# mohsij/spacecraft-pose-estimation

Measured on AMD Instinct MI355X. Metric: poses/sec end-to-end (HRNet+PnP) at batch 256; keypoint/pose err vs ref, higher is better.
Workload: dtype bf16

## Files before the change

### spacecraft-pose-estimation_amd/csrc/bottleneck.hip

```cpp
#include "common.h"
#include "conv_device.h"
#include "conv_pipe_kernel.h"

namespace scpose {

namespace {

constexpr int kT = 16;
constexpr int kHW = kT + 2, kHPix = kHW * kHW;
constexpr int kCols1 = (kHPix + 15) / 16;
constexpr int kXS = (kHPix | 1) * 16;
constexpr int kT2S = (kT * kT | 1) * 16;
constexpr int kW1Bytes = 8 * 4 * 4 * 16 * 16;
constexpr int kW2LSteps = 13;
constexpr int kLds = 8 * kXS + 8 * kT2S + kW1Bytes + (64 + 64 + 256) * 4 + 16 + kW2LSteps * 4 * 1024;
constexpr int kW1BytesProj = 2 * 4 * 4 * 16 * 16;
constexpr int kLdsProj = 8 * kXS + 8 * kT2S + 2 * 8 * kT2S + kW1BytesProj + (64 + 64 + 256) * 4 + 16;

struct BneckLaunch {
  const void* in;
  const void* w1;
  const void* w2;
  const void* w3;
  const float* b1;
  const float* b2;
  const float* b3;
  void* out;
  uint32_t in_bytes, out_bytes;
  int32_t N, H, W;
  int32_t tiles_x, tiles_y, tiles_total, grid;
  uint32_t* sched;
  int32_t xcd_local;
  unsigned long long* dbg_buf;
};

inline int bneck_row_channel(int row) {
  const int q = row >> 2, reg = row & 3;
  return (q & 1) * 8 + (q >> 1) * 4 + reg;
}

}

template <int S, int E, typename F>
__device__ __forceinline__ void static_for_b(F&& f) {
  if constexpr (S < E) { f(std::integral_constant<int, S>{}); static_for_b<S + 1, E>(f); }
}

#ifndef SCPOSE_BNECK_EARLY
#define SCPOSE_BNECK_EARLY 2
#endif
#ifndef SCPOSE_BNECK_EARLY_PROJ
#define SCPOSE_BNECK_EARLY_PROJ 1
#endif
template <int DT, bool PROJ>
__global__ __launch_bounds__(512, 2) void bottleneck_kernel(const BneckLaunch p) {
  constexpr int EARLY = PROJ ? SCPOSE_BNECK_EARLY_PROJ : SCPOSE_BNECK_EARLY;
  constexpr int CINP = PROJ ? 8 : 32;
  constexpr int KA = CINP / 4;
  constexpr int KC = PROJ ? 4 : 2;
  constexpr int W1B = PROJ ? kW1BytesProj : kW1Bytes;
  extern __shared__ __attribute__((aligned(16))) char smem[];
  typedef typename DtOf<DT>::type T;
  typedef typename FragOf<T>::type frag_t;
  char* t1l = smem;
  char* t2l = t1l + 8 * kXS;
  char* xcl = t2l + 8 * kT2S;
  char* w1l = xcl + (PROJ ? 2 * 8 * kT2S : 0);

  const int tid = threadIdx.x, lane = tid & 63, wave = __builtin_amdgcn_readfirstlane(tid >> 6);
  const int q = lane >> 4, r = lane & 15, half = lane >> 5, psel = q & 1;
  const int ch = wave & 1, wq = wave >> 1;
  const int HW = p.H * p.W;
  const int tiles_per_img = p.tiles_x * p.tiles_y;

  for (int o = tid * 16; o < W1B; o += 512 * 16)
    *reinterpret_cast<u32x4*>(w1l + o) = *reinterpret_cast<const u32x4*>(static_cast<const char*>(p.w1) + o);
  frag_t w3f[KC][2];
#pragma unroll
  for (int s = 0; s < KC; ++s)
#pragma unroll
    for (int mb = 0; mb < 2; ++mb)
      w3f[s][mb] = *reinterpret_cast<const frag_t*>(static_cast<const char*>(p.w3) + ((((size_t)s * 16 + 2 * wave + mb) * 4 + q) * 16 + r) * 16);
  float* bl = reinterpret_cast<float*>(w1l + W1B);
  for (int e = tid; e < 64 + 64 + 256; e += 512) bl[e] = e < 64 ? p.b1[e] : e < 128 ? p.b2[e - 64] : p.b3[e - 128];
  const int qoff = q * kXS;
  const uint32_t w2vo = (uint32_t)(((2 * ch) * 4 + q) * 16 + r) * 16u;

  int* tq = reinterpret_cast<int*>(bl + 64 + 64 + 256);
  constexpr int W2L = PROJ ? 0 : kW2LSteps;
  char* w2ll = reinterpret_cast<char*>(tq) + 16;
  for (int o = tid * 16; o < W2L * 4 * 1024; o += 512 * 16)
    *reinterpret_cast<u32x4*>(w2ll + o) = *reinterpret_cast<const u32x4*>(static_cast<const char*>(p.w2) + o);
  const int xcd = xcc_id();
  auto claim = [&]() { return p.xcd_local ? tile_claim_xcd(p.sched, xcd, p.N, tiles_per_img) : tile_claim(p.sched + 9, p.tiles_total); };
  if (tid == 0) { tq[0] = claim(); tq[1] = tq[0] < 0 ? -1 : claim(); }
  __syncthreads();
  int t = tq[0], t_next = tq[1];
  auto decode = [&](int t, int& img, int& oy0, int& ox0) {
    img = t / tiles_per_img;
    const int rem = t - img * tiles_per_img;
    const int ty = rem / p.tiles_x;
    oy0 = ty * kT; ox0 = (rem - ty * p.tiles_x) * kT;
  };
  const buf_rsrc_t rs_in = make_buf(p.in, p.in_bytes), rs_out = make_buf(p.out, p.out_bytes), rs_w2 = make_buf(p.w2, 18u * 4 * 4 * 16 * 16);
  const uint32_t kstep_bytes = (uint32_t)(4 * HW) * 16u;

  const bool has_col2 = wave + 16 < kCols1;
  uint32_t vo[3];
  int cx[3] = {-1, -1, -1};
  auto locate = [&](int t) {
    int img, oy0, ox0;
    decode(t, img, oy0, ox0);
#pragma unroll
    for (int i = 0; i < 3; ++i) {
      const int slot = (wave + 8 * i) * 16 + r;
      const int my = slot / kHW, mx = slot - my * kHW;
      const int gy = oy0 - 1 + my, gx = ox0 - 1 + mx;
      const bool ok = slot < kHPix && gy >= 0 && gy < p.H && gx >= 0 && gx < p.W;
      vo[i] = ok ? (uint32_t)((img * CINP + q) * HW + gy * p.W + gx) * 16u : BUF_OOB;
      if constexpr (PROJ) cx[i] = (slot < kHPix && my >= 1 && my <= kT && mx >= 1 && mx <= kT) ? ((my - 1) * kT + mx - 1) * 16 : -1;
    }
  };
  u32x4 xr[KA][3];
  auto request = [&](auto sc) {
    constexpr int S = decltype(sc)::value;
    if constexpr (S < KA)
#pragma unroll
      for (int i = 0; i < 3; ++i)
        xr[S][i] = load16_buf(rs_in, vo[i], (uint32_t)S * kstep_bytes);
  };
  auto request_head = [&]() {
    request(std::integral_constant<int, 0>{}); request(std::integral_constant<int, 1>{});
    request(std::integral_constant<int, 2>{}); request(std::integral_constant<int, 3>{});
    request(std::integral_constant<int, 4>{}); request(std::integral_constant<int, 5>{});
    request(std::integral_constant<int, 6>{}); request(std::integral_constant<int, 7>{});
  };

  if (t >= 0) {
    locate(t);
    request_head();
  }
  asm volatile("s_waitcnt lgkmcnt(0)" ::: "memory");
  __builtin_amdgcn_s_barrier();

  unsigned long long tph[6] = {0, 0, 0, 0, 0, 0};
  auto now = [&]() -> unsigned long long { return SCP_DBG_BUF(p) ? __builtin_amdgcn_s_memtime() : 0ull; };
  int xbuf = 0;
  for (; t >= 0; t = t_next, t_next = tq[2], xbuf ^= 1) {
    int img, oy0, ox0;
    decode(t, img, oy0, ox0);
    const unsigned long long ts0 = now();
    int t_after = -1;
    if (tid == 0 && t_next >= 0) t_after = claim();

    frag_t w2f[18 - W2L][2];
    const uint32_t pl_bytes = (uint32_t)HW * 16u;
    auto out_off = [&](int cp) -> uint32_t {
      const int oy = oy0 + 2 * cp + half, ox = ox0 + r;
      return (oy < p.H && ox < p.W) ? (uint32_t)((img * 32 + psel) * HW + oy * p.W + ox) * 16u : BUF_OOB;
    };
    u32x4 rv[PROJ ? 1 : 8][2];
    {
      f32x4 acc[4][3];
#pragma unroll
      for (int mb = 0; mb < 4; ++mb) {
        const float4 bs = *reinterpret_cast<const float4*>(bl + mb * 16 + q * 4);
        acc[mb][0] = f32x4{bs.x, bs.y, bs.z, bs.w}; acc[mb][1] = acc[mb][0]; acc[mb][2] = acc[mb][0];
      }
      auto load_a = [&](int s, frag_t* a) {
#pragma unroll
        for (int mb = 0; mb < 4; ++mb) a[mb] = *reinterpret_cast<const frag_t*>(w1l + ((((s * 4 + mb) * 4 + q) * 16 + r) * 16));
      };
      frag_t fa[2][4];
      load_a(0, fa[0]);
      auto step = [&](auto sc) {
        constexpr int S = decltype(sc)::value;
        if constexpr (S + 1 < KA) load_a(S + 1, fa[(S + 1) & 1]);
        if constexpr (PROJ) {
#pragma unroll
          for (int i = 0; i < 3; ++i)
            if (cx[i] >= 0) *reinterpret_cast<u32x4*>(xcl + (xbuf * 8 + 4 * S + q) * kT2S + cx[i]) = xr[S][i];
        }
        __builtin_amdgcn_sched_barrier(0);
#pragma unroll
        for (int mb = 0; mb < 4; ++mb) {
          acc[mb][0] = mfma16<T>(fa[S & 1][mb], __builtin_bit_cast(frag_t, xr[S][0]), acc[mb][0]);
          acc[mb][1] = mfma16<T>(fa[S & 1][mb], __builtin_bit_cast(frag_t, xr[S][1]), acc[mb][1]);
          if (has_col2) acc[mb][2] = mfma16<T>(fa[S & 1][mb], __builtin_bit_cast(frag_t, xr[S][2]), acc[mb][2]);
        }
        __builtin_amdgcn_sched_barrier(0);
      };
      step(std::integral_constant<int, 0>{}); step(std::integral_constant<int, 1>{});
      if constexpr (KA > 2) {
        step(std::integral_constant<int, 2>{}); step(std::integral_constant<int, 3>{}); step(std::integral_constant<int, 4>{});
        step(std::integral_constant<int, 5>{}); step(std::integral_constant<int, 6>{}); step(std::integral_constant<int, 7>{});
      }
#pragma unroll
      for (int i = 0; i < 3; ++i) {
        const int slot = (wave + 8 * i) * 16 + r;
        const bool inimg = vo[i] != BUF_OOB;
#pragma unroll
        for (int mb = 0; mb < 4; ++mb) {
          uint2 o;
          o.x = relu2_16(pack2<T>(acc[mb][i][0], acc[mb][i][1]), 0u);
          o.y = relu2_16(pack2<T>(acc[mb][i][2], acc[mb][i][3]), 0u);
          if (!inimg) o = make_uint2(0u, 0u);
          if (slot < kHPix) *reinterpret_cast<uint2*>(t1l + (2 * mb + psel) * kXS + slot * 16 + 8 * (q >> 1)) = o;
        }
      }
      __builtin_amdgcn_sched_barrier(0);
#pragma unroll
      for (int s2 = W2L; s2 < 18; ++s2)
#pragma unroll
        for (int mb = 0; mb < 2; ++mb)
          w2f[s2 - W2L][mb] = __builtin_bit_cast(frag_t, load16_buf(rs_w2, w2vo, (uint32_t)((s2 * 4 + mb) * 1024)));
      __builtin_amdgcn_sched_barrier(0);
      if constexpr (!PROJ) {
#pragma unroll
        for (int cp = 0; cp < 8; ++cp) {
          const uint32_t o = out_off(cp);
#pragma unroll
          for (int mb = 0; mb < 2; ++mb) rv[cp][mb] = load16_buf(rs_in, o, (uint32_t)(2 * (2 * wave + mb)) * pl_bytes);
        }
        __builtin_amdgcn_sched_barrier(0);
      }
    }
    const unsigned long long ts1 = now();
    asm volatile("s_waitcnt lgkmcnt(0)" ::: "memory");
    __builtin_amdgcn_s_barrier();
    const unsigned long long ts2 = now();

    if constexpr (EARLY > 0) {
      __builtin_amdgcn_sched_barrier(0);
      if (t_next >= 0) locate(t_next);
      else { vo[0] = vo[1] = vo[2] = BUF_OOB; cx[0] = cx[1] = cx[2] = -1; }
      static_for_b<0, EARLY>([&](auto sc) { request(sc); });
      __builtin_amdgcn_sched_barrier(0);
    }
    constexpr int CC = PROJ ? 1 : 2;
#pragma unroll 1
    for (int c0 = 0; c0 < 4; c0 += CC) {
      f32x4 acc[2][CC];
#pragma unroll
      for (int mb = 0; mb < 2; ++mb) {
        const float4 bs = *reinterpret_cast<const float4*>(bl + 64 + (2 * ch + mb) * 16 + q * 4);
#pragma unroll
        for (int cc = 0; cc < CC; ++cc) acc[mb][cc] = f32x4{bs.x, bs.y, bs.z, bs.w};
      }
      const int px = r;
      const char* bq0 = t1l + ((wq + 4 * c0) * kHW + px) * 16 + qoff;
      const char* aq0 = w2ll + (2 * ch) * 1024 + lane * 16;
      auto k2imm = [](int s) { const int tap = s >> 1, ky = tap / 3, kx = tap - 3 * ky; return 4 * (s & 1) * kXS + (ky * kHW + kx) * 16; };
      frag_t bq[3][CC], aq[3][2];
      auto fetch = [&](auto sc) {
        constexpr int S = decltype(sc)::value;
        if constexpr (S < 18) {
#pragma unroll
          for (int cc = 0; cc < CC; ++cc) bq[S % 3][cc] = *reinterpret_cast<const frag_t*>(bq0 + cc * (4 * kHW * 16) + k2imm(S));
          if constexpr (S < W2L) {
            aq[S % 3][0] = *reinterpret_cast<const frag_t*>(aq0 + S * 4096);
            aq[S % 3][1] = *reinterpret_cast<const frag_t*>(aq0 + S * 4096 + 1024);
          }
        }
      };
      fetch(std::integral_constant<int, 0>{});
      fetch(std::integral_constant<int, 1>{});
      auto kstep = [&](auto sc) {
        constexpr int S = decltype(sc)::value;
        fetch(std::integral_constant<int, S + 2>{});
        __builtin_amdgcn_sched_barrier(0);
#pragma unroll
        for (int mb = 0; mb < 2; ++mb) {
          frag_t a;
          if constexpr (S < W2L) a = aq[S % 3][mb]; else a = w2f[S - W2L][mb];
#pragma unroll
          for (int cc = 0; cc < CC; ++cc) acc[mb][cc] = mfma16<T>(a, bq[S % 3][cc], acc[mb][cc]);
        }
        __builtin_amdgcn_sched_barrier(0);
      };
      kstep(std::integral_constant<int, 0>{}); kstep(std::integral_constant<int, 1>{}); kstep(std::integral_constant<int, 2>{});
      kstep(std::integral_constant<int, 3>{}); kstep(std::integral_constant<int, 4>{}); kstep(std::integral_constant<int, 5>{});
      kstep(std::integral_constant<int, 6>{}); kstep(std::integral_constant<int, 7>{}); kstep(std::integral_constant<int, 8>{});
      kstep(std::integral_constant<int, 9>{}); kstep(std::integral_constant<int, 10>{}); kstep(std::integral_constant<int, 11>{});
      kstep(std::integral_constant<int, 12>{}); kstep(std::integral_constant<int, 13>{}); kstep(std::integral_constant<int, 14>{});
      kstep(std::integral_constant<int, 15>{}); kstep(std::integral_constant<int, 16>{}); kstep(std::integral_constant<int, 17>{});
#pragma unroll
      for (int cc = 0; cc < CC; ++cc) {
        const int pix = (wq + 4 * (c0 + cc)) * kT + px;
#pragma unroll
        for (int mb = 0; mb < 2; ++mb) {
          uint2 o;
          o.x = relu2_16(pack2<T>(acc[mb][cc][0], acc[mb][cc][1]), 0u);
          o.y = relu2_16(pack2<T>(acc[mb][cc][2], acc[mb][cc][3]), 0u);
          *reinterpret_cast<uint2*>(t2l + (2 * (2 * ch + mb) + psel) * kT2S + pix * 16 + 8 * (q >> 1)) = o;
        }
      }
    }
    const unsigned long long ts3 = now();
    if (tid == 0) tq[2] = t_after;
    asm volatile("s_waitcnt lgkmcnt(0)" ::: "memory");
    __builtin_amdgcn_s_barrier();
    const unsigned long long ts4 = now();

    {
      __builtin_amdgcn_sched_barrier(0);
      if constexpr (EARLY == 0) {
        if (t_next >= 0) locate(t_next);
        else { vo[0] = vo[1] = vo[2] = BUF_OOB; cx[0] = cx[1] = cx[2] = -1; }
      }
      auto pair = [&](auto cpc) {
        constexpr int cp = decltype(cpc)::value;
        request(std::integral_constant<int, cp + EARLY>{});
        f32x4 acc[2][2];
#pragma unroll
        for (int mb = 0; mb < 2; ++mb) {
          const float4 bs = *reinterpret_cast<const float4*>(bl + 128 + (2 * wave + mb) * 16 + q * 4);
          acc[mb][0] = f32x4{bs.x, bs.y, bs.z, bs.w}; acc[mb][1] = acc[mb][0];
        }
        frag_t bc[KC][2];
#pragma unroll
        for (int s = 0; s < KC; ++s)
#pragma unroll
          for (int c = 0; c < 2; ++c)
            bc[s][c] = *reinterpret_cast<const frag_t*>((s < 2 ? t2l + (4 * s + q) * kT2S : xcl + (xbuf * 8 + 4 * (s - 2) + q) * kT2S) + ((2 * cp + c) * 16 + r) * 16);
        __builtin_amdgcn_sched_barrier(0);
#pragma unroll
        for (int s = 0; s < KC; ++s)
#pragma unroll
          for (int mb = 0; mb < 2; ++mb)
#pragma unroll
            for (int c = 0; c < 2; ++c) acc[mb][c] = mfma16<T>(w3f[s][mb], bc[s][c], acc[mb][c]);
        mfma_swap_pad(acc[0][0], acc[0][1], acc[1][0], acc[1][1]);
#pragma unroll
        for (int mb = 0; mb < 2; ++mb) {
          const f32x4 a0 = acc[mb][0], a1 = acc[mb][1];
          uint32_t a[4], b[4];
#pragma unroll
          for (int jj = 0; jj < 4; ++jj) { a[jj] = __float_as_uint(a0[jj]); b[jj] = __float_as_uint(a1[jj]); }
#pragma unroll
          for (int jj = 0; jj < 4; ++jj) {
            const auto sw = __builtin_amdgcn_permlane32_swap(a[jj], b[jj], false, false);
            a[jj] = sw[0]; b[jj] = sw[1];
          }
          float v[8];
#pragma unroll
          for (int jj = 0; jj < 4; ++jj) { v[jj] = __uint_as_float(a[jj]); v[4 + jj] = __uint_as_float(b[jj]); }
          if constexpr (!PROJ) {
          const u32x4 rr = rv[cp][mb];
          v[0] += from_bits<T>(rr[0] & 0xffff); v[1] += from_bits<T>(rr[0] >> 16);
          v[2] += from_bits<T>(rr[1] & 0xffff); v[3] += from_bits<T>(rr[1] >> 16);
          v[4] += from_bits<T>(rr[2] & 0xffff); v[5] += from_bits<T>(rr[2] >> 16);
          v[6] += from_bits<T>(rr[3] & 0xffff); v[7] += from_bits<T>(rr[3] >> 16);
          }
          u32x4 ov;
          ov[0] = relu2_16(pack2<T>(v[0], v[1]), 0u); ov[1] = relu2_16(pack2<T>(v[2], v[3]), 0u);
          ov[2] = relu2_16(pack2<T>(v[4], v[5]), 0u); ov[3] = relu2_16(pack2<T>(v[6], v[7]), 0u);
          store16_buf(rs_out, out_off(cp), (uint32_t)(2 * (2 * wave + mb)) * pl_bytes, ov);
        }
      };
      pair(std::integral_constant<int, 0>{}); pair(std::integral_constant<int, 1>{}); pair(std::integral_constant<int, 2>{});
      pair(std::integral_constant<int, 3>{}); pair(std::integral_constant<int, 4>{}); pair(std::integral_constant<int, 5>{});
      pair(std::integral_constant<int, 6>{}); pair(std::integral_constant<int, 7>{});
    }
    if (SCP_DBG_BUF(p)) {
      const unsigned long long ts5 = now();
      tph[0] += ts1 - ts0; tph[1] += ts2 - ts1; tph[2] += ts3 - ts2; tph[3] += ts4 - ts3; tph[4] += ts5 - ts4;
    }
  }
  if (tid == 0) { if (p.xcd_local) tile_retire_xcd(p.sched); else tile_retire(p.sched + 9); }
  if (SCP_DBG_BUF(p) && lane == 0)
    for (int k = 0; k < 6; ++k) SCP_DBG_BUF(p)[((size_t)blockIdx.x * 8 + wave) * 6 + k] = tph[k];
}

bool bottleneck_fusable(int cin, int cmid, int cout) { return (cin == 256 || cin == 64) && cmid == 64 && cout == 256; }

void bottleneck_pack(const float* w1, const float* w2, const float* w3, const float* wds, const float* b1, const float* b2, const float* b3,
                     const float* bds, int cin, int dtype,
                     std::vector<uint16_t>* pw1, std::vector<uint16_t>* pw2, std::vector<uint16_t>* pw3, std::vector<float>* pb) {
  const int ka = cin / 32, kc = wds ? 4 : 2;
  pw1->assign((size_t)ka * 4 * 4 * 16 * 8, 0);
  pw2->assign((size_t)18 * 4 * 4 * 16 * 8, 0);
  pw3->assign((size_t)kc * 16 * 4 * 16 * 8, 0);
  pb->assign(64 + 64 + 256, 0.f);
  for (int s = 0; s < ka; ++s)
    for (int m = 0; m < 4; ++m)
      for (int q = 0; q < 4; ++q)
        for (int r = 0; r < 16; ++r) {
          const int co = 16 * m + bneck_row_channel(r), plane = 4 * s + q;
          uint16_t* d = pw1->data() + ((((size_t)s * 4 + m) * 4 + q) * 16 + r) * 8;
          for (int j = 0; j < 8; ++j) d[j] = host_f32_to_16(w1[(size_t)co * cin + plane * 8 + j], dtype);
        }
  for (int s = 0; s < 18; ++s)
    for (int m = 0; m < 4; ++m)
      for (int q = 0; q < 4; ++q)
        for (int r = 0; r < 16; ++r) {
          const int co = 16 * m + bneck_row_channel(r);
          const int t = 4 * s + q, tap = t >> 3, plane = t & 7, ky = tap / 3, kx = tap % 3;
          uint16_t* d = pw2->data() + ((((size_t)s * 4 + m) * 4 + q) * 16 + r) * 8;
          for (int j = 0; j < 8; ++j) d[j] = host_f32_to_16(w2[((size_t)(co * 64 + plane * 8 + j) * 3 + ky) * 3 + kx], dtype);
        }
  for (int s = 0; s < kc; ++s)
    for (int m = 0; m < 16; ++m)
      for (int q = 0; q < 4; ++q)
        for (int r = 0; r < 16; ++r) {
          const int co = 16 * m + bneck_row_channel(r), plane = 4 * s + q;
          uint16_t* d = pw3->data() + ((((size_t)s * 16 + m) * 4 + q) * 16 + r) * 8;
          const float* src = plane < 8 ? w3 + (size_t)co * 64 + plane * 8 : wds + (size_t)co * 64 + (plane - 8) * 8;
          for (int j = 0; j < 8; ++j) d[j] = host_f32_to_16(src[j], dtype);
        }
  for (int pos = 0; pos < 64; ++pos) {
    const int co = (pos & ~15) + bneck_row_channel(pos & 15);
    (*pb)[pos] = b1[co]; (*pb)[64 + pos] = b2[co];
  }
  for (int pos = 0; pos < 256; ++pos) {
    const int co = (pos & ~15) + bneck_row_channel(pos & 15);
    (*pb)[128 + pos] = b3[co] + (bds ? bds[co] : 0.f);
  }
}

template <int DT, bool PROJ>
static int32_t bneck_launch_one(const BneckLaunch& L, hipStream_t stream) {
  auto kern = bottleneck_kernel<DT, PROJ>;
  constexpr int lds = PROJ ? kLdsProj : kLds;
  static LdsOptIn big;
  { const int32_t rc = lds_opt_in(reinterpret_cast<const void*>(kern), lds, &big); if (rc != SCPOSE_OK) return rc; }
  hipLaunchKernelGGL(kern, dim3(L.grid), dim3(512), lds, stream, L);
  SCP_CHECK_HIP(hipGetLastError());
  return SCPOSE_OK;
}

int32_t bottleneck_launch(const void* in, const void* w1, const void* w2, const void* w3, const float* bias, int N, int H, int W,
                          int cin, int dtype, void* out, uint32_t* sched, hipStream_t stream) {
  SCP_REQUIRE(sched, "bottleneck: null tile-queue words");
  const bool proj = cin == 64;
  SCP_REQUIRE(cin == 64 || cin == 256, "bottleneck: Cin = %d (64 or 256)", cin);
  const size_t in_frame = blocked_bytes(1, cin / 8, H, W), out_frame = blocked_bytes(1, 32, H, W);
  return for_frame_ranges(N, out_frame, [&](int n0, int n) -> int32_t {
    BneckLaunch L{};
    L.in = static_cast<const char*>(in) + (size_t)n0 * in_frame;
    L.out = static_cast<char*>(out) + (size_t)n0 * out_frame;
    L.w1 = w1; L.w2 = w2; L.w3 = w3; L.b1 = bias; L.b2 = bias + 64; L.b3 = bias + 128;
    L.in_bytes = (uint32_t)((size_t)n * in_frame); L.out_bytes = (uint32_t)((size_t)n * out_frame);
    L.N = n; L.H = H; L.W = W;
    L.tiles_x = (W + kT - 1) / kT; L.tiles_y = (H + kT - 1) / kT;
    L.tiles_total = n * L.tiles_x * L.tiles_y;
    L.grid = conv_device_cus() < L.tiles_total ? conv_device_cus() : L.tiles_total;
    L.sched = sched;
    { static const char* e = dev_env("SCPOSE_BNECK_GLOBALQ"); L.xcd_local = !(e && atoi(e)); }
    { static const char* e = dev_env("SCPOSE_BNECK_DBG"); L.dbg_buf = (kDevBuild && e && atoi(e)) ? conv_dbg_buffer(stream) : nullptr; if (L.dbg_buf) conv_dbg_set_grid(L.grid); }
    if (dtype == SCPOSE_DT_BF16) return proj ? bneck_launch_one<0, true>(L, stream) : bneck_launch_one<0, false>(L, stream);
    return proj ? bneck_launch_one<1, true>(L, stream) : bneck_launch_one<1, false>(L, stream);
  }, "bottleneck %d %dx%d", cin, H, W);
}

}
```

Before: 9994.

## Split bottleneck kernel into projection and identity paths, reuse centre input for residual

The fused bottleneck kernel is split into a projection variant and a specialised identity variant. The identity path splits input loads into centre pixels and halo ring, and keeps the centre registers for the residual add instead of reloading the input. It also prefetches the next tile's centre inputs inside the conv3 loop and stages w3 in LDS. Part of w2 moves from LDS to registers, and the conv2 wave/tile mapping changes to 4 output blocks by 2 row groups. The trade-off is more register pressure and a new LDS layout. An env override for grid size is also added.

```diff
diff --git a/spacecraft-pose-estimation_amd/csrc/bottleneck.hip b/spacecraft-pose-estimation_amd/csrc/bottleneck.hip
--- a/spacecraft-pose-estimation_amd/csrc/bottleneck.hip
+++ b/spacecraft-pose-estimation_amd/csrc/bottleneck.hip
@@ -12,8 +12,11 @@
 constexpr int kXS = (kHPix | 1) * 16;
 constexpr int kT2S = (kT * kT | 1) * 16;
 constexpr int kW1Bytes = 8 * 4 * 4 * 16 * 16;
-constexpr int kW2LSteps = 13;
-constexpr int kLds = 8 * kXS + 8 * kT2S + kW1Bytes + (64 + 64 + 256) * 4 + 16 + kW2LSteps * 4 * 1024;
+constexpr int kW3Bytes = 2 * 16 * 4 * 16 * 16;
+constexpr int kW2LSteps = 5;
+constexpr int kRing = 4 * kT + 4;
+constexpr int kLds = 8 * kXS + 8 * kT2S + kW1Bytes + (64 + 64 + 256) * 4 + 16 + kW2LSteps * 4 * 1024 + kW3Bytes;
+static_assert(kLds <= 160 * 1024, "identity Bottleneck: LDS");
 constexpr int kW1BytesProj = 2 * 4 * 4 * 16 * 16;
 constexpr int kLdsProj = 8 * kXS + 8 * kT2S + 2 * 8 * kT2S + kW1BytesProj + (64 + 64 + 256) * 4 + 16;
 
@@ -46,26 +49,23 @@
   if constexpr (S < E) { f(std::integral_constant<int, S>{}); static_for_b<S + 1, E>(f); }
 }
 
-#ifndef SCPOSE_BNECK_EARLY
-#define SCPOSE_BNECK_EARLY 2
-#endif
 #ifndef SCPOSE_BNECK_EARLY_PROJ
 #define SCPOSE_BNECK_EARLY_PROJ 1
 #endif
-template <int DT, bool PROJ>
-__global__ __launch_bounds__(512, 2) void bottleneck_kernel(const BneckLaunch p) {
-  constexpr int EARLY = PROJ ? SCPOSE_BNECK_EARLY_PROJ : SCPOSE_BNECK_EARLY;
-  constexpr int CINP = PROJ ? 8 : 32;
+template <int DT>
+__device__ __forceinline__ void bneck_first(const BneckLaunch& p) {
+  constexpr int EARLY = SCPOSE_BNECK_EARLY_PROJ;
+  constexpr int CINP = 8;
   constexpr int KA = CINP / 4;
-  constexpr int KC = PROJ ? 4 : 2;
-  constexpr int W1B = PROJ ? kW1BytesProj : kW1Bytes;
+  constexpr int KC = 4;
+  constexpr int W1B = kW1BytesProj;
   extern __shared__ __attribute__((aligned(16))) char smem[];
   typedef typename DtOf<DT>::type T;
   typedef typename FragOf<T>::type frag_t;
   char* t1l = smem;
   char* t2l = t1l + 8 * kXS;
   char* xcl = t2l + 8 * kT2S;
-  char* w1l = xcl + (PROJ ? 2 * 8 * kT2S : 0);
+  char* w1l = xcl + 2 * 8 * kT2S;
 
   const int tid = threadIdx.x, lane = tid & 63, wave = __builtin_amdgcn_readfirstlane(tid >> 6);
   const int q = lane >> 4, r = lane & 15, half = lane >> 5, psel = q & 1;
@@ -87,10 +87,6 @@
   const uint32_t w2vo = (uint32_t)(((2 * ch) * 4 + q) * 16 + r) * 16u;
 
   int* tq = reinterpret_cast<int*>(bl + 64 + 64 + 256);
-  constexpr int W2L = PROJ ? 0 : kW2LSteps;
-  char* w2ll = reinterpret_cast<char*>(tq) + 16;
-  for (int o = tid * 16; o < W2L * 4 * 1024; o += 512 * 16)
-    *reinterpret_cast<u32x4*>(w2ll + o) = *reinterpret_cast<const u32x4*>(static_cast<const char*>(p.w2) + o);
   const int xcd = xcc_id();
   auto claim = [&]() { return p.xcd_local ? tile_claim_xcd(p.sched, xcd, p.N, tiles_per_img) : tile_claim(p.sched + 9, p.tiles_total); };
   if (tid == 0) { tq[0] = claim(); tq[1] = tq[0] < 0 ? -1 : claim(); }
@@ -118,7 +114,7 @@
       const int gy = oy0 - 1 + my, gx = ox0 - 1 + mx;
       const bool ok = slot < kHPix && gy >= 0 && gy < p.H && gx >= 0 && gx < p.W;
       vo[i] = ok ? (uint32_t)((img * CINP + q) * HW + gy * p.W + gx) * 16u : BUF_OOB;
-      if constexpr (PROJ) cx[i] = (slot < kHPix && my >= 1 && my <= kT && mx >= 1 && mx <= kT) ? ((my - 1) * kT + mx - 1) * 16 : -1;
+      cx[i] = (slot < kHPix && my >= 1 && my <= kT && mx >= 1 && mx <= kT) ? ((my - 1) * kT + mx - 1) * 16 : -1;
     }
   };
   u32x4 xr[KA][3];
@@ -153,13 +149,12 @@
     int t_after = -1;
     if (tid == 0 && t_next >= 0) t_after = claim();
 
-    frag_t w2f[18 - W2L][2];
+    frag_t w2f[18][2];
     const uint32_t pl_bytes = (uint32_t)HW * 16u;
     auto out_off = [&](int cp) -> uint32_t {
       const int oy = oy0 + 2 * cp + half, ox = ox0 + r;
       return (oy < p.H && ox < p.W) ? (uint32_t)((img * 32 + psel) * HW + oy * p.W + ox) * 16u : BUF_OOB;
     };
-    u32x4 rv[PROJ ? 1 : 8][2];
     {
       f32x4 acc[4][3];
 #pragma unroll
@@ -176,11 +171,9 @@
       auto step = [&](auto sc) {
         constexpr int S = decltype(sc)::value;
         if constexpr (S + 1 < KA) load_a(S + 1, fa[(S + 1) & 1]);
-        if constexpr (PROJ) {
-#pragma unroll
-          for (int i = 0; i < 3; ++i)
-            if (cx[i] >= 0) *reinterpret_cast<u32x4*>(xcl + (xbuf * 8 + 4 * S + q) * kT2S + cx[i]) = xr[S][i];
-        }
+#pragma unroll
+        for (int i = 0; i < 3; ++i)
+          if (cx[i] >= 0) *reinterpret_cast<u32x4*>(xcl + (xbuf * 8 + 4 * S + q) * kT2S + cx[i]) = xr[S][i];
         __builtin_amdgcn_sched_barrier(0);
 #pragma unroll
         for (int mb = 0; mb < 4; ++mb) {
@@ -190,11 +183,8 @@
         }
         __builtin_amdgcn_sched_barrier(0);
       };
+      static_assert(KA == 2, "two k-steps of conv1");
       step(std::integral_constant<int, 0>{}); step(std::integral_constant<int, 1>{});
-      if constexpr (KA > 2) {
-        step(std::integral_constant<int, 2>{}); step(std::integral_constant<int, 3>{}); step(std::integral_constant<int, 4>{});
-        step(std::integral_constant<int, 5>{}); step(std::integral_constant<int, 6>{}); step(std::integral_constant<int, 7>{});
-      }
 #pragma unroll
       for (int i = 0; i < 3; ++i) {
         const int slot = (wave + 8 * i) * 16 + r;
@@ -210,20 +200,11 @@
       }
       __builtin_amdgcn_sched_barrier(0);
 #pragma unroll
-      for (int s2 = W2L; s2 < 18; ++s2)
+      for (int s2 = 0; s2 < 18; ++s2)
 #pragma unroll
         for (int mb = 0; mb < 2; ++mb)
-          w2f[s2 - W2L][mb] = __builtin_bit_cast(frag_t, load16_buf(rs_w2, w2vo, (uint32_t)((s2 * 4 + mb) * 1024)));
-      __builtin_amdgcn_sched_barrier(0);
-      if constexpr (!PROJ) {
-#pragma unroll
-        for (int cp = 0; cp < 8; ++cp) {
-          const uint32_t o = out_off(cp);
-#pragma unroll
-          for (int mb = 0; mb < 2; ++mb) rv[cp][mb] = load16_buf(rs_in, o, (uint32_t)(2 * (2 * wave + mb)) * pl_bytes);
-        }
-        __builtin_amdgcn_sched_barrier(0);
-      }
+          w2f[s2][mb] = __builtin_bit_cast(frag_t, load16_buf(rs_w2, w2vo, (uint32_t)((s2 * 4 + mb) * 1024)));
+      __builtin_amdgcn_sched_barrier(0);
     }
     const unsigned long long ts1 = now();
     asm volatile("s_waitcnt lgkmcnt(0)" ::: "memory");
@@ -237,7 +218,7 @@
       static_for_b<0, EARLY>([&](auto sc) { request(sc); });
       __builtin_amdgcn_sched_barrier(0);
     }
-    constexpr int CC = PROJ ? 1 : 2;
+    constexpr int CC = 1;
 #pragma unroll 1
     for (int c0 = 0; c0 < 4; c0 += CC) {
       f32x4 acc[2][CC];
@@ -249,18 +230,13 @@
       }
       const int px = r;
       const char* bq0 = t1l + ((wq + 4 * c0) * kHW + px) * 16 + qoff;
-      const char* aq0 = w2ll + (2 * ch) * 1024 + lane * 16;
       auto k2imm = [](int s) { const int tap = s >> 1, ky = tap / 3, kx = tap - 3 * ky; return 4 * (s & 1) * kXS + (ky * kHW + kx) * 16; };
-      frag_t bq[3][CC], aq[3][2];
+      frag_t bq[3][CC];
       auto fetch = [&](auto sc) {
         constexpr int S = decltype(sc)::value;
         if constexpr (S < 18) {
 #pragma unroll
           for (int cc = 0; cc < CC; ++cc) bq[S % 3][cc] = *reinterpret_cast<const frag_t*>(bq0 + cc * (4 * kHW * 16) + k2imm(S));
-          if constexpr (S < W2L) {
-            aq[S % 3][0] = *reinterpret_cast<const frag_t*>(aq0 + S * 4096);
-            aq[S % 3][1] = *reinterpret_cast<const frag_t*>(aq0 + S * 4096 + 1024);
-          }
         }
       };
       fetch(std::integral_constant<int, 0>{});
@@ -271,10 +247,8 @@
         __builtin_amdgcn_sched_barrier(0);
 #pragma unroll
         for (int mb = 0; mb < 2; ++mb) {
-          frag_t a;
-          if constexpr (S < W2L) a = aq[S % 3][mb]; else a = w2f[S - W2L][mb];
-#pragma unroll
-          for (int cc = 0; cc < CC; ++cc) acc[mb][cc] = mfma16<T>(a, bq[S % 3][cc], acc[mb][cc]);
+#pragma unroll
+          for (int cc = 0; cc < CC; ++cc) acc[mb][cc] = mfma16<T>(w2f[S][mb], bq[S % 3][cc], acc[mb][cc]);
         }
         __builtin_amdgcn_sched_barrier(0);
       };
@@ -345,22 +319,275 @@
           float v[8];
 #pragma unroll
           for (int jj = 0; jj < 4; ++jj) { v[jj] = __uint_as_float(a[jj]); v[4 + jj] = __uint_as_float(b[jj]); }
-          if constexpr (!PROJ) {
-          const u32x4 rr = rv[cp][mb];
+          u32x4 ov;
+          ov[0] = relu2_16(pack2<T>(v[0], v[1]), 0u); ov[1] = relu2_16(pack2<T>(v[2], v[3]), 0u);
+          ov[2] = relu2_16(pack2<T>(v[4], v[5]), 0u); ov[3] = relu2_16(pack2<T>(v[6], v[7]), 0u);
+          store16_buf(rs_out, out_off(cp), (uint32_t)(2 * (2 * wave + mb)) * pl_bytes, ov);
+        }
+      };
+      pair(std::integral_constant<int, 0>{}); pair(std::integral_constant<int, 1>{}); pair(std::integral_constant<int, 2>{});
+      pair(std::integral_constant<int, 3>{}); pair(std::integral_constant<int, 4>{}); pair(std::integral_constant<int, 5>{});
+      pair(std::integral_constant<int, 6>{}); pair(std::integral_constant<int, 7>{});
+    }
+    if (SCP_DBG_BUF(p)) {
+      const unsigned long long ts5 = now();
+      tph[0] += ts1 - ts0; tph[1] += ts2 - ts1; tph[2] += ts3 - ts2; tph[3] += ts4 - ts3; tph[4] += ts5 - ts4;
+    }
+  }
+  if (tid == 0) { if (p.xcd_local) tile_retire_xcd(p.sched); else tile_retire(p.sched + 9); }
+  if (SCP_DBG_BUF(p) && lane == 0)
+    for (int k = 0; k < 6; ++k) SCP_DBG_BUF(p)[((size_t)blockIdx.x * 8 + wave) * 6 + k] = tph[k];
+}
+
+template <int DT>
+__device__ __forceinline__ void bneck_identity(const BneckLaunch& p) {
+  constexpr int KA = 8;
+  constexpr int W2L = kW2LSteps;
+  extern __shared__ __attribute__((aligned(16))) char smem[];
+  typedef typename DtOf<DT>::type T;
+  typedef typename FragOf<T>::type frag_t;
+  char* t1l = smem;
+  char* t2l = t1l + 8 * kXS;
+  char* w1l = t2l + 8 * kT2S;
+  float* bl = reinterpret_cast<float*>(w1l + kW1Bytes);
+  int* tq = reinterpret_cast<int*>(bl + 64 + 64 + 256);
+  char* w2ll = reinterpret_cast<char*>(tq) + 16;
+  char* w3l = w2ll + W2L * 4 * 1024;
+
+  const int tid = threadIdx.x, lane = tid & 63, wave = __builtin_amdgcn_readfirstlane(tid >> 6);
+  const int q = lane >> 4, r = lane & 15, psel = q & 1;
+  const int blk = wave & 3, rg = wave >> 2;
+  const int HW = p.H * p.W;
+  const int tiles_per_img = p.tiles_x * p.tiles_y;
+
+  for (int o = tid * 16; o < kW1Bytes; o += 512 * 16)
+    *reinterpret_cast<u32x4*>(w1l + o) = *reinterpret_cast<const u32x4*>(static_cast<const char*>(p.w1) + o);
+  for (int o = tid * 16; o < W2L * 4 * 1024; o += 512 * 16)
+    *reinterpret_cast<u32x4*>(w2ll + o) = *reinterpret_cast<const u32x4*>(static_cast<const char*>(p.w2) + o);
+  for (int o = tid * 16; o < kW3Bytes; o += 512 * 16)
+    *reinterpret_cast<u32x4*>(w3l + o) = *reinterpret_cast<const u32x4*>(static_cast<const char*>(p.w3) + o);
+  for (int e = tid; e < 64 + 64 + 256; e += 512) bl[e] = e < 64 ? p.b1[e] : e < 128 ? p.b2[e - 64] : p.b3[e - 128];
+  const int qoff = q * kXS;
+  const uint32_t w2vo = (uint32_t)(blk * 1024 + lane * 16);
+
+  const int xcd = xcc_id();
+  auto claim = [&]() { return p.xcd_local ? tile_claim_xcd(p.sched, xcd, p.N, tiles_per_img) : tile_claim(p.sched + 9, p.tiles_total); };
+  if (tid == 0) { tq[0] = claim(); tq[1] = tq[0] < 0 ? -1 : claim(); }
+  __syncthreads();
+  int t = tq[0], t_next = tq[1];
+  const buf_rsrc_t rs_in = make_buf(p.in, p.in_bytes), rs_out = make_buf(p.out, p.out_bytes), rs_w2 = make_buf(p.w2, 18u * 4 * 4 * 16 * 16);
+  const uint32_t kstep_bytes = (uint32_t)(4 * HW) * 16u;
+
+  const bool has_col2 = wave < (kRing + 15) / 16;
+  const int rj = wave * 16 + r;
+  const bool ring_ok = rj < kRing;
+  const int ring_my = rj < kHW ? 0 : rj < 2 * kHW ? kHW - 1 : rj < 2 * kHW + kT ? rj - (2 * kHW - 1) : rj - (2 * kHW + kT - 1);
+  const int ring_mx = rj < kHW ? rj : rj < 2 * kHW ? rj - kHW : rj < 2 * kHW + kT ? 0 : kHW - 1;
+  const int slot[3] = {(wave + 1) * kHW + r + 1, (wave + 9) * kHW + r + 1, ring_ok ? ring_my * kHW + ring_mx : 0};
+  uint32_t vo[3];
+  auto locate = [&](int t) {
+    const int img = t / tiles_per_img;
+    const int rem = t - img * tiles_per_img;
+    const int ty = rem / p.tiles_x;
+    const int oy0 = ty * kT, ox0 = (rem - ty * p.tiles_x) * kT;
+#pragma unroll
+    for (int i = 0; i < 3; ++i) {
+      const int my = i == 0 ? wave + 1 : i == 1 ? wave + 9 : ring_my, mx = i < 2 ? r + 1 : ring_mx;
+      const int gy = oy0 - 1 + my, gx = ox0 - 1 + mx;
+      const bool ok = (i < 2 || ring_ok) && gy >= 0 && gy < p.H && gx >= 0 && gx < p.W;
+      vo[i] = ok ? (uint32_t)((img * 32 + q) * HW + gy * p.W + gx) * 16u : BUF_OOB;
+    }
+  };
+  u32x4 xr[KA][3];
+  auto request_centre = [&](auto sc) {
+    constexpr int S = decltype(sc)::value;
+    xr[S][0] = load16_buf(rs_in, vo[0], (uint32_t)S * kstep_bytes);
+    xr[S][1] = load16_buf(rs_in, vo[1], (uint32_t)S * kstep_bytes);
+  };
+  auto request_ring = [&](auto sc) {
+    constexpr int S = decltype(sc)::value;
+    xr[S][2] = load16_buf(rs_in, vo[2], (uint32_t)S * kstep_bytes);
+  };
+  if (t >= 0) {
+    locate(t);
+    static_for_b<0, KA>([&](auto sc) { request_centre(sc); request_ring(sc); });
+  }
+  asm volatile("s_waitcnt lgkmcnt(0)" ::: "memory");
+  __builtin_amdgcn_s_barrier();
+
+  unsigned long long tph[6] = {0, 0, 0, 0, 0, 0};
+  auto now = [&]() -> unsigned long long { return SCP_DBG_BUF(p) ? __builtin_amdgcn_s_memtime() : 0ull; };
+  for (; t >= 0; t = t_next, t_next = tq[2]) {
+    const unsigned long long ts0 = now();
+    int t_after = -1;
+    if (tid == 0 && t_next >= 0) t_after = claim();
+
+    frag_t w2f[18 - W2L];
+    {
+      f32x4 acc[4][3];
+#pragma unroll
+      for (int mb = 0; mb < 4; ++mb) {
+        const float4 bs = *reinterpret_cast<const float4*>(bl + mb * 16 + q * 4);
+        acc[mb][0] = f32x4{bs.x, bs.y, bs.z, bs.w}; acc[mb][1] = acc[mb][0]; acc[mb][2] = acc[mb][0];
+      }
+      auto load_a = [&](int s, frag_t* a) {
+#pragma unroll
+        for (int mb = 0; mb < 4; ++mb) a[mb] = *reinterpret_cast<const frag_t*>(w1l + ((((s * 4 + mb) * 4 + q) * 16 + r) * 16));
+      };
+      frag_t fa[2][4];
+      load_a(0, fa[0]);
+      static_for_b<0, KA>([&](auto sc) {
+        constexpr int S = decltype(sc)::value;
+        if constexpr (S + 1 < KA) load_a(S + 1, fa[(S + 1) & 1]);
+        __builtin_amdgcn_sched_barrier(0);
+#pragma unroll
+        for (int mb = 0; mb < 4; ++mb) {
+          acc[mb][0] = mfma16<T>(fa[S & 1][mb], __builtin_bit_cast(frag_t, xr[S][0]), acc[mb][0]);
+          acc[mb][1] = mfma16<T>(fa[S & 1][mb], __builtin_bit_cast(frag_t, xr[S][1]), acc[mb][1]);
+          if (has_col2) acc[mb][2] = mfma16<T>(fa[S & 1][mb], __builtin_bit_cast(frag_t, xr[S][2]), acc[mb][2]);
+        }
+        __builtin_amdgcn_sched_barrier(0);
+      });
+#pragma unroll
+      for (int i = 0; i < 3; ++i) {
+        const bool inimg = vo[i] != BUF_OOB;
+        const bool mine = i < 2 || (has_col2 && ring_ok);
+#pragma unroll
+        for (int mb = 0; mb < 4; ++mb) {
+          uint2 o;
+          o.x = relu2_16(pack2<T>(acc[mb][i][0], acc[mb][i][1]), 0u);
+          o.y = relu2_16(pack2<T>(acc[mb][i][2], acc[mb][i][3]), 0u);
+          if (!inimg) o = make_uint2(0u, 0u);
+          if (mine) *reinterpret_cast<uint2*>(t1l + (2 * mb + psel) * kXS + slot[i] * 16 + 8 * (q >> 1)) = o;
+        }
+      }
+      __builtin_amdgcn_sched_barrier(0);
+#pragma unroll
+      for (int s2 = W2L; s2 < 18; ++s2) w2f[s2 - W2L] = __builtin_bit_cast(frag_t, load16_buf(rs_w2, w2vo, (uint32_t)(s2 * 4096)));
+      __builtin_amdgcn_sched_barrier(0);
+    }
+    const unsigned long long ts1 = now();
+    asm volatile("s_waitcnt lgkmcnt(0)" ::: "memory");
+    __builtin_amdgcn_s_barrier();
+    const unsigned long long ts2 = now();
+
+    const uint32_t co[2] = {vo[0], vo[1]};
+    __builtin_amdgcn_sched_barrier(0);
+    if (t_next >= 0) locate(t_next);
+    else vo[0] = vo[1] = vo[2] = BUF_OOB;
+    static_for_b<0, KA>([&](auto sc) { request_ring(sc); });
+    __builtin_amdgcn_sched_barrier(0);
+    constexpr int CC = 2;
+#pragma unroll 1
+    for (int c0 = 0; c0 < 8; c0 += CC) {
+      f32x4 acc[CC];
+      {
+        const float4 bs = *reinterpret_cast<const float4*>(bl + 64 + blk * 16 + q * 4);
+#pragma unroll
+        for (int cc = 0; cc < CC; ++cc) acc[cc] = f32x4{bs.x, bs.y, bs.z, bs.w};
+      }
+      const int px = r;
+      const char* bq0 = t1l + ((rg + 2 * c0) * kHW + px) * 16 + qoff;
+      const char* aq0 = w2ll + blk * 1024 + lane * 16;
+      auto k2imm = [](int s) { const int tap = s >> 1, ky = tap / 3, kx = tap - 3 * ky; return 4 * (s & 1) * kXS + (ky * kHW + kx) * 16; };
+      frag_t bq[3][CC], aq[3];
+      auto fetch = [&](auto sc) {
+        constexpr int S = decltype(sc)::value;
+        if constexpr (S < 18) {
+#pragma unroll
+          for (int cc = 0; cc < CC; ++cc) bq[S % 3][cc] = *reinterpret_cast<const frag_t*>(bq0 + cc * (2 * kHW * 16) + k2imm(S));
+          if constexpr (S < W2L) aq[S % 3] = *reinterpret_cast<const frag_t*>(aq0 + S * 4096);
+        }
+      };
+      fetch(std::integral_constant<int, 0>{});
+      fetch(std::integral_constant<int, 1>{});
+      static_for_b<0, 18>([&](auto sc) {
+        constexpr int S = decltype(sc)::value;
+        fetch(std::integral_constant<int, S + 2>{});
+        __builtin_amdgcn_sched_barrier(0);
+        frag_t a;
+        if constexpr (S < W2L) a = aq[S % 3]; else a = w2f[S - W2L];
+#pragma unroll
+        for (int cc = 0; cc < CC; ++cc) acc[cc] = mfma16<T>(a, bq[S % 3][cc], acc[cc]);
+        __builtin_amdgcn_sched_barrier(0);
+      });
+#pragma unroll
+      for (int cc = 0; cc < CC; ++cc) {
+        const int pix = (rg + 2 * (c0 + cc)) * kT + px;
+        uint2 o;
+        o.x = relu2_16(pack2<T>(acc[cc][0], acc[cc][1]), 0u);
+        o.y = relu2_16(pack2<T>(acc[cc][2], acc[cc][3]), 0u);
+        *reinterpret_cast<uint2*>(t2l + (2 * blk + psel) * kT2S + pix * 16 + 8 * (q >> 1)) = o;
+      }
+    }
+    const unsigned long long ts3 = now();
+    if (tid == 0) tq[2] = t_after;
+    asm volatile("s_waitcnt lgkmcnt(0)" ::: "memory");
+    __builtin_amdgcn_s_barrier();
+    const unsigned long long ts4 = now();
+
+    {
+      __builtin_amdgcn_sched_barrier(0);
+      frag_t bt[2][2];
+#pragma unroll
+      for (int s = 0; s < 2; ++s)
+#pragma unroll
+        for (int i = 0; i < 2; ++i) bt[s][i] = *reinterpret_cast<const frag_t*>(t2l + (4 * s + q) * kT2S + ((wave + 8 * i) * kT + r) * 16);
+      auto load_w3 = [&](int S, frag_t (*a)[2]) {
+#pragma unroll
+        for (int s = 0; s < 2; ++s)
+#pragma unroll
+          for (int mb = 0; mb < 2; ++mb) a[s][mb] = *reinterpret_cast<const frag_t*>(w3l + (s * 16 + 2 * S + mb) * 1024 + lane * 16);
+      };
+      frag_t fw[2][2][2];
+      load_w3(0, fw[0]);
+      static_for_b<0, KA>([&](auto sc) {
+        constexpr int S = decltype(sc)::value;
+        if constexpr (S + 1 < KA) load_w3(S + 1, fw[(S + 1) & 1]);
+        f32x4 acc[2][2];
+#pragma unroll
+        for (int mb = 0; mb < 2; ++mb) {
+          const float4 bs = *reinterpret_cast<const float4*>(bl + 128 + (2 * S + mb) * 16 + q * 4);
+          acc[mb][0] = f32x4{bs.x, bs.y, bs.z, bs.w}; acc[mb][1] = acc[mb][0];
+        }
+        __builtin_amdgcn_sched_barrier(0);
+#pragma unroll
+        for (int s = 0; s < 2; ++s)
+#pragma unroll
+          for (int mb = 0; mb < 2; ++mb)
+#pragma unroll
+            for (int i = 0; i < 2; ++i) acc[mb][i] = mfma16<T>(fw[S & 1][s][mb], bt[s][i], acc[mb][i]);
+        mfma_swap_pad(acc[0][0], acc[0][1], acc[1][0], acc[1][1]);
+        u32x4 ov[2];
+#pragma unroll
+        for (int i = 0; i < 2; ++i) {
+          const f32x4 a0 = acc[0][i], a1 = acc[1][i];
+          uint32_t a[4], b[4];
+#pragma unroll
+          for (int jj = 0; jj < 4; ++jj) { a[jj] = __float_as_uint(a0[jj]); b[jj] = __float_as_uint(a1[jj]); }
+#pragma unroll
+          for (int jj = 0; jj < 4; ++jj) {
+            const auto sw = __builtin_amdgcn_permlane32_swap(a[jj], b[jj], false, false);
+            a[jj] = sw[0]; b[jj] = sw[1];
+          }
+          float v[8];
+#pragma unroll
+          for (int jj = 0; jj < 4; ++jj) { v[jj] = __uint_as_float(a[jj]); v[4 + jj] = __uint_as_float(b[jj]); }
+          const u32x4 rr = xr[S][i];
           v[0] += from_bits<T>(rr[0] & 0xffff); v[1] += from_bits<T>(rr[0] >> 16);
           v[2] += from_bits<T>(rr[1] & 0xffff); v[3] += from_bits<T>(rr[1] >> 16);
           v[4] += from_bits<T>(rr[2] & 0xffff); v[5] += from_bits<T>(rr[2] >> 16);
           v[6] += from_bits<T>(rr[3] & 0xffff); v[7] += from_bits<T>(rr[3] >> 16);
-          }
-          u32x4 ov;
-          ov[0] = relu2_16(pack2<T>(v[0], v[1]), 0u); ov[1] = relu2_16(pack2<T>(v[2], v[3]), 0u);
-          ov[2] = relu2_16(pack2<T>(v[4], v[5]), 0u); ov[3] = relu2_16(pack2<T>(v[6], v[7]), 0u);
-          store16_buf(rs_out, out_off(cp), (uint32_t)(2 * (2 * wave + mb)) * pl_bytes, ov);
-        }
-      };
-      pair(std::integral_constant<int, 0>{}); pair(std::integral_constant<int, 1>{}); pair(std::integral_constant<int, 2>{});
-      pair(std::integral_constant<int, 3>{}); pair(std::integral_constant<int, 4>{}); pair(std::integral_constant<int, 5>{});
-      pair(std::integral_constant<int, 6>{}); pair(std::integral_constant<int, 7>{});
+          ov[i][0] = relu2_16(pack2<T>(v[0], v[1]), 0u); ov[i][1] = relu2_16(pack2<T>(v[2], v[3]), 0u);
+          ov[i][2] = relu2_16(pack2<T>(v[4], v[5]), 0u); ov[i][3] = relu2_16(pack2<T>(v[6], v[7]), 0u);
+        }
+        __builtin_amdgcn_sched_barrier(0);
+        request_centre(sc);
+        __builtin_amdgcn_sched_barrier(0);
+        store16_buf(rs_out, co[0], (uint32_t)S * kstep_bytes, ov[0]);
+        store16_buf(rs_out, co[1], (uint32_t)S * kstep_bytes, ov[1]);
+        __builtin_amdgcn_sched_barrier(0);
+      });
     }
     if (SCP_DBG_BUF(p)) {
       const unsigned long long ts5 = now();
@@ -370,6 +597,12 @@
   if (tid == 0) { if (p.xcd_local) tile_retire_xcd(p.sched); else tile_retire(p.sched + 9); }
   if (SCP_DBG_BUF(p) && lane == 0)
     for (int k = 0; k < 6; ++k) SCP_DBG_BUF(p)[((size_t)blockIdx.x * 8 + wave) * 6 + k] = tph[k];
+}
+
+template <int DT, bool PROJ>
+__global__ __launch_bounds__(512, 2) void bottleneck_kernel(const BneckLaunch p) {
+  if constexpr (PROJ) bneck_first<DT>(p);
+  else bneck_identity<DT>(p);
 }
 
 bool bottleneck_fusable(int cin, int cmid, int cout) { return (cin == 256 || cin == 64) && cmid == 64 && cout == 256; }
@@ -447,6 +680,7 @@
     L.grid = conv_device_cus() < L.tiles_total ? conv_device_cus() : L.tiles_total;
     L.sched = sched;
     { static const char* e = dev_env("SCPOSE_BNECK_GLOBALQ"); L.xcd_local = !(e && atoi(e)); }
+    { static const char* e = dev_env("SCPOSE_BNECK_GRID"); if (e && atoi(e) > 0 && atoi(e) < L.grid) L.grid = atoi(e); }
     { static const char* e = dev_env("SCPOSE_BNECK_DBG"); L.dbg_buf = (kDevBuild && e && atoi(e)) ? conv_dbg_buffer(stream) : nullptr; if (L.dbg_buf) conv_dbg_set_grid(L.grid); }
     if (dtype == SCPOSE_DT_BF16) return proj ? bneck_launch_one<0, true>(L, stream) : bneck_launch_one<0, false>(L, stream);
     return proj ? bneck_launch_one<1, true>(L, stream) : bneck_launch_one<1, false>(L, stream);
```

Result: no change. 10030 (median of 6 runs) (+0.4%).
